# LordLiang/DrawingSpinUp

Hardware: AMD Instinct MI355X
Metric: drawings/sec end-to-end (512x512, 6 views, 24 frames) (higher is better)
Workload: dtype f16 (diffusion) / f16 table + f32 MLP (NSR) / f32 (stage-1 deformable convolutions, IS-Net, contour) / f32 with bf16 x 3 products (stage-2 convolutions; the reference: cuDNN TF32)

## Files before the change

drawingspinup_amd/_lib.py:

```python
import ctypes as C
import os

import torch

_HERE = os.path.dirname(os.path.abspath(__file__))
LIB_PATH = os.environ.get("DSU_HIP_LIB") or os.path.join(_HERE, "libdsu_hip.so")
MAX_LEVELS = 16

c_i32, c_i64, c_u32, c_f32, c_vp = C.c_int32, C.c_int64, C.c_uint32, C.c_float, C.c_void_p


class HashGridCfg(C.Structure):
    _fields_ = [("n_levels", c_u32), ("n_features", c_u32), ("log2_hashmap_size", c_u32),
                ("base_resolution", c_u32), ("per_level_scale", C.c_double)]


class HashGridLevels(C.Structure):
    _fields_ = [("offsets", c_u32 * (MAX_LEVELS + 1)), ("resolution", c_u32 * MAX_LEVELS),
                ("scale", c_f32 * MAX_LEVELS), ("hashed", c_u32 * MAX_LEVELS)]


class SdfMlp(C.Structure):
    _fields_ = [("w0", c_vp), ("b0", c_vp), ("w1", c_vp), ("b1", c_vp)]

# ... 158 lines not shown
    "dsu_nsr_driver_sync": [c_vp],
    "dsu_nsr_driver_timing": [c_vp, c_i32],
    "dsu_nsr_driver_timing_read": [c_vp, c_i32, C.POINTER(c_i64), C.POINTER(C.c_double),
                                   C.POINTER(C.c_double)],
    "dsu_nsr_driver_timing_flops": [c_vp, c_i32, C.POINTER(C.c_double)],
    "dsu_spatial_sort": [P, c_i64, c_f32, c_i32, P, P, P, c_i64, P],
    "dsu_spatial_sort_workspace_bytes": [c_i64, c_i32],
    "dsu_ray_aabb": [P, P, c_i64, P, P, c_f32, P, P, P],
    "dsu_ray_march_count": [P, P, P, P, c_i64, P, P, c_i32, c_f32, P, P],
    "dsu_ray_march_fill": [P, P, P, P, c_i64, P, P, c_i32, c_f32, P, P, P, P, P],
    "dsu_ray_march_scratch": [P, P, P, P, c_i64, P, P, c_i32, c_f32, c_i32, P, P, P, P],
    "dsu_ray_compact": [P, P, c_i32, P, P, c_i64, P, P, P, P],
    "dsu_ray_compact_points": [P, P, c_i32, P, P, c_i64, P, P, P, P, P, P],
    "dsu_ray_compact_points_cap": [P, P, c_i32, P, P, c_i64, P, P, P, P, P, c_i64, P],
    "dsu_points_tail": [P, c_i64, P, P, P, c_i64, c_f32, P],
    "dsu_spatial_sort_dev": [P, c_i64, P, c_i64, c_f32, c_i32, P, P, P, c_i64, P],
    "dsu_ray_offsets": [P, c_i64, P, P, P],
    "dsu_ortho_ray_batch": [P, P, P, c_i64, P, P, P, P, c_i32, P, P, P, c_i32, c_i32, P, P, P, P, P,
                            P, P],
    "dsu_ortho_ray_batch_split": [P, P, P, c_i64, P, P, P, P, c_i32, P, P, P, c_i32, c_i32, P, P, P, P, P,
                            P, P, P, P],
    "dsu_ray_losses": [P, P, P, P, P, P, c_i32, C.POINTER(RayLossCfg), P, P, P],
    "dsu_sample_losses": [P, P, c_i64, c_i64, c_f32, c_f32, c_f32, c_f32, c_i32, P, P, P, P],
    "dsu_texture_fwd": [C.POINTER(TexMlp), P, c_i64, P, P],
    "dsu_texture_bwd_workspace_bytes": [c_i64],
    "dsu_texture_bwd": [C.POINTER(TexMlp), P, P, P, c_i64, P, P, P, P, P, P, P, P, c_i64, P],
    "dsu_texture_fwd_shaded": [C.POINTER(TexMlp), P, P, c_i64, P, P, P],
    "dsu_texture_bwd_shaded": [C.POINTER(TexMlp), P, P, P, P, P, c_i64, c_i64, P, P, P, P, P, P, P, P,
                               P, c_i64, P],
    "dsu_weights_from_alpha_fwd": [P, P, P, c_i64, P, P],
    "dsu_weights_from_alpha_bwd": [P, P, P, P, P, c_i64, P, P],
    "dsu_accumulate_fwd": [P, P, c_i32, P, P, c_i64, P, P],
    "dsu_neus_composite_fwd": [P, P, P, P, P, P, P, P, c_i64, P, c_f32, P, P, P, P],
    "dsu_neus_composite_bwd": [P, P, P, P, P, P, P, P, c_i64, P, c_f32, P, P, P, P, P, P, P,
                               P, P],
    "dsu_shade_prep_fwd": [P, P, c_i64, P, P, P],
    "dsu_shade_prep_bwd": [P, P, P, c_i64, P, P, P],
    "dsu_shade_prep_bwd_tail": [P, P, P, c_i64, c_i64, P, P, P],
    "dsu_occgrid_ema": [P, P, P, c_i64, c_f32, P, P],
    "dsu_occgrid_binarize": [P, c_i64, c_f32, P, P],
    "dsu_ric_offsets": [c_i32, c_i32, P, P],
    "dsu_deform_conv3x3_fwd": [P, P, c_i64, P, c_i32, c_i32, c_i32, c_i32, c_i32, c_i32, P, P,
                               c_i32, P, P, P],
    "dsu_mv_attention_fwd": [P, P, P, P, P, c_i32, c_i32, c_i32, c_i32, c_i32, c_i32,
                             C.POINTER(c_i64), C.POINTER(c_i64), C.POINTER(c_i64),
                             C.POINTER(c_i64), c_f32, P],
# ... 113 lines not shown
```

drawingspinup_amd/csrc/nsr_driver.hip:

```cpp
#include "common.h"
#include "adamw_dev.h"

#include <math.h>
#include <string.h>

#include <mutex>
#include <vector>

namespace {

constexpr int N_GEO = 64 * 23 + 64 + 13 * 64 + 13;
constexpr int N_TEX = 64 * 16 + 64 + 64 * 64 + 64 + 3 * 64 + 3;
constexpr int N_SMALL = (64 * 23 + 64 + 64) + (13 * 64 + 13 + 13) + N_TEX + 1;

__device__ __forceinline__ uint4 philox(uint4 c, uint2 k) {
#pragma unroll
  for (int i = 0; i < 10; ++i) {
    const uint32_t hi0 = __umulhi(0xD2511F53u, c.x), lo0 = 0xD2511F53u * c.x;
    const uint32_t hi1 = __umulhi(0xCD9E8D57u, c.z), lo1 = 0xCD9E8D57u * c.z;
    c = make_uint4(hi1 ^ c.y ^ k.x, lo1, hi0 ^ c.w ^ k.y, lo0);
    k.x += 0x9E3779B9u;
    k.y += 0xBB67AE85u;
  }
  return c;
// ... 38 lines not shown
  float* variance;
  float* g_geo;
  float* g_tex;
  float* d_inv;
  float *m, *v;
  float *w0_eff, *w1_eff, *inv_s;
  float* zero_terms;
  const float* terms;
  float* terms_out;
  float lr_geo, lr_tex, lr_var, beta1, beta2, eps, wd, bc1, bc2_sqrt;
  int32_t update;
};

__device__ __forceinline__ void adamw_elem(float& x, float g, float& m, float& v, float lr,
                                           const SmallArgs& a) {
  const float omb1 = (float)(1.0 - (double)a.beta1), omb2 = (float)(1.0 - (double)a.beta2);
  x -= lr * a.wd * x;
  m = m + (g - m) * omb1;
  v = a.beta2 * v + omb2 * g * g;
  const float denom = sqrtf(v) / a.bc2_sqrt + a.eps;
  x -= (lr / a.bc1) * m / denom;
}

__global__ __launch_bounds__(1024) void small_update_kernel(SmallArgs a, dsu_table_adamw_args ta) {
  if (blockIdx.x > 0) {
    dsu_table_adamw_range(ta, (int64_t)(blockIdx.x - 1) * 1024 + threadIdx.x,
                          (int64_t)(gridDim.x - 1) * 1024);
    return;
  }
  __shared__ float s_g[N_GEO];
  __shared__ float s_v0[64 * 23], s_v1[13 * 64];
  __shared__ float s_gain[77], s_norm[77], s_dot[77];
  const int t = threadIdx.x;
  for (int i = t; i < 64 * 23; i += 1024) s_v0[i] = a.w0_v[i];
  for (int i = t; i < 13 * 64; i += 1024) s_v1[i] = a.w1_v[i];
  if (t < 77) s_gain[t] = t < 64 ? a.w0_g[t] : a.w1_g[t - 64];
  if (a.update)
    for (int i = t; i < N_GEO; i += 1024) s_g[i] = a.g_geo[i];
  __syncthreads();
  if (a.update) {
    if (t < 77) {
      const bool l0 = t < 64;
      const int r = l0 ? t : t - 64, cols = l0 ? 23 : 64;
      const float* vrow = (l0 ? s_v0 : s_v1) + r * cols;
      const float* grow = (l0 ? s_g : s_g + 64 * 23 + 64) + r * cols;
      float nn = 0.0f, dot = 0.0f;
      for (int c = 0; c < cols; ++c) {
        nn += vrow[c] * vrow[c];
        dot += grow[c] * vrow[c];
      }
      s_norm[t] = sqrtf(nn);
      s_dot[t] = dot;
    }
    __syncthreads();
    int off = 0;
    for (int i = t; i < 64 * 23; i += 1024) {
      const int r = i / 23;
      const float nrm = s_norm[r];
      const float g = (s_gain[r] / nrm) * (s_g[i] - s_v0[i] * s_dot[r] / (nrm * nrm));
      float x = s_v0[i], m = a.m[off + i], v = a.v[off + i];
      adamw_elem(x, g, m, v, a.lr_geo, a);
      a.w0_v[i] = x; a.m[off + i] = m; a.v[off + i] = v;
      s_v0[i] = x;
    }
    off += 64 * 23;
    float new_gain = 0.0f;
    if (t < 64) {
      float x = s_gain[t], m = a.m[off + t], v = a.v[off + t];
      adamw_elem(x, s_dot[t] / s_norm[t], m, v, a.lr_geo, a);
      a.w0_g[t] = x; a.m[off + t] = m; a.v[off + t] = v;
      new_gain = x;
    }
    off += 64;
    if (t < 64) {
      float x = a.b0[t], m = a.m[off + t], v = a.v[off + t];
      adamw_elem(x, s_g[64 * 23 + t], m, v, a.lr_geo, a);
      a.b0[t] = x; a.m[off + t] = m; a.v[off + t] = v;
    }
    off += 64;
    for (int i = t; i < 13 * 64; i += 1024) {
      const int r = i / 64;
      const float nrm = s_norm[64 + r];
      const float g = (s_gain[64 + r] / nrm) *
                      (s_g[64 * 23 + 64 + i] - s_v1[i] * s_dot[64 + r] / (nrm * nrm));
      float x = s_v1[i], m = a.m[off + i], v = a.v[off + i];
      adamw_elem(x, g, m, v, a.lr_geo, a);
      a.w1_v[i] = x; a.m[off + i] = m; a.v[off + i] = v;
      s_v1[i] = x;
    }
    off += 13 * 64;
    float new_gain1 = 0.0f;
    if (t < 13) {
      float x = s_gain[64 + t], m = a.m[off + t], v = a.v[off + t];
      adamw_elem(x, s_dot[64 + t] / s_norm[64 + t], m, v, a.lr_geo, a);
      a.w1_g[t] = x; a.m[off + t] = m; a.v[off + t] = v;
      new_gain1 = x;
    }
    off += 13;
    if (t < 13) {
      float x = a.b1[t], m = a.m[off + t], v = a.v[off + t];
      adamw_elem(x, s_g[64 * 23 + 64 + 13 * 64 + t], m, v, a.lr_geo, a);
      a.b1[t] = x; a.m[off + t] = m; a.v[off + t] = v;
    }
    off += 13;
    const int tn[6] = {64 * 16, 64, 64 * 64, 64, 3 * 64, 3};
    int go = 0;
    for (int k = 0; k < 6; ++k) {
      float* p = a.tex[k];
      for (int i = t; i < tn[k]; i += 1024) {
        float x = p[i], m = a.m[off + i], v = a.v[off + i];
        adamw_elem(x, a.g_tex[go + i], m, v, a.lr_tex, a);
        p[i] = x; a.m[off + i] = m; a.v[off + i] = v;
      }
      off += tn[k];
      go += tn[k];
    }
    if (t == 1023) {
      float x = a.variance[0], m = a.m[off], v = a.v[off];
      const float g = a.d_inv[0] * expf(x * 10.0f) * 10.0f;
      adamw_elem(x, g, m, v, a.lr_var, a);
      a.variance[0] = x; a.m[off] = m; a.v[off] = v;
      a.inv_s[0] = expf(x * 10.0f);
      a.d_inv[0] = 0.0f;
    }
    if (t < 3) a.zero_terms[t] = 0.0f;
    if (t >= 8 && t < 16 && a.terms_out) a.terms_out[t - 8] = a.terms[t - 8];
    __syncthreads();
    if (t < 64) s_gain[t] = new_gain;
    if (t < 13) s_gain[64 + t] = new_gain1;
    for (int i = t; i < N_GEO; i += 1024) a.g_geo[i] = 0.0f;
    for (int i = t; i < N_TEX; i += 1024) a.g_tex[i] = 0.0f;
    __syncthreads();
  } else if (t == 1023) {
    a.inv_s[0] = expf(a.variance[0] * 10.0f);
  }
  if (t < 77) {
    const bool l0 = t < 64;
    const int r = l0 ? t : t - 64, cols = l0 ? 23 : 64;
    const float* vrow = (l0 ? s_v0 : s_v1) + r * cols;
    float nn = 0.0f;
    for (int c = 0; c < cols; ++c) nn += vrow[c] * vrow[c];
    s_norm[t] = s_gain[t] / sqrtf(nn);
  }
  __syncthreads();
  for (int i = t; i < 64 * 23; i += 1024) a.w0_eff[i] = s_v0[i] * s_norm[i / 23];
  for (int i = t; i < 13 * 64; i += 1024) a.w1_eff[i] = s_v1[i] * s_norm[64 + i / 64];
}

struct Carve {
  char* base;
  int64_t off = 0;
  template <typename T>
  T* take(int64_t count) {
    off = (off + 255) / 256 * 256;
    T* p = base ? reinterpret_cast<T*>(base + off) : nullptr;
    off += count * (int64_t)sizeof(T);
    return p;
// ... 245 lines not shown
  sa.lr_geo = sa.lr_tex = sa.lr_var = 0.0f;
  sa.bc1 = sa.bc2_sqrt = 1.0f;
  if (update) {
    sa.lr_geo = a->lr_geometry; sa.lr_tex = a->lr_texture; sa.lr_var = a->lr_variance;
    sa.bc1 = (float)(1.0 - pow((double)c.beta1, (double)a->adam_step));
    sa.bc2_sqrt = (float)sqrt(1.0 - pow((double)c.beta2, (double)a->adam_step));
  }
  dsu_table_adamw_args ta{};
  int table_blocks = 0;
  if (update && a->table_p && !d->fold) {
    DSU_TRY(dsu_table_adamw(a->table_p, a->table_grad, a->table_m, a->table_v,
                            const_cast<void*>(a->table_img), a->table_n, a->table_lr, c.beta1, c.beta2,
                            a->table_eps, a->table_wd, a->table_bc1, a->table_bc2_sqrt, s));
  } else if (update && a->table_p) {
    if (a->table_n < 0 || (a->table_n & 3) || !a->table_grad || !a->table_m || !a->table_v ||
        !a->table_img || !(a->table_bc1 > 0.0f) || !(a->table_bc2_sqrt > 0.0f))
      return DSU_EINVAL;
    ta = dsu_table_adamw_args{(float4*)a->table_p, (float4*)a->table_grad, (float4*)a->table_m,
                              (float4*)a->table_v, (__half2*)const_cast<void*>(a->table_img),
                              a->table_n / 4, a->table_lr, c.beta1, c.beta2, a->table_eps,
                              a->table_wd, a->table_bc1, a->table_bc2_sqrt};
    table_blocks = (int)((ta.n4 + 1023) / 1024 < 512 ? (ta.n4 + 1023) / 1024 : 512);
  }
  small_update_kernel<<<dim3(1 + table_blocks), dim3(1024), 0, s>>>(sa, ta);
  DSU_CHECK_LAUNCH();
  return DSU_OK;
}

}

extern "C" {

int dsu_nsr_draws(uint64_t seed, int64_t step, int32_t n_rays, int32_t V, int32_t H, int32_t W,
                  int64_t* index, int64_t* x, int64_t* y, float* jitter, int32_t n_random,
                  float* pts_random, float* perturb, void* stream) {
  if (n_rays < 0 || n_random < 0 || V < 1 || H < 1 || W < 1 ||
      (n_rays && (!index || !x || !y || !jitter)) || (n_random && (!pts_random || !perturb)))
    return DSU_EINVAL;
  const int n = n_rays > n_random ? n_rays : n_random;
  if (n == 0) return DSU_OK;
  nsr_draw_kernel<<<dim3((n + 255) / 256), dim3(256), 0, (hipStream_t)stream>>>(
      seed, step, n_rays, V, H, W, index, x, y, jitter, n_random, pts_random, perturb);
  DSU_CHECK_LAUNCH();
  return DSU_OK;
}

int64_t dsu_nsr_driver_workspace_bytes(const dsu_nsr_driver_cfg* cfg) {
// ... 169 lines not shown
  if (d->timing) { d->work[0] += alg_bytes; d->flops[0] += fwd_flops; }
  if (a->prefetch_next && d->pack_gate == 1) {
    const int q = (int)((a->step + 1) % 3);
    dsu_nsr_step_args na = *a;
    na.inj_index = na.inj_x = na.inj_y = nullptr;
    na.inj_jitter = na.inj_pts_random = na.inj_perturb = nullptr;
    na.inj_rays = nullptr;
    DSU_HIP(hipEventRecord(d->fwd_done, s));
    DSU_HIP(hipStreamWaitEvent(d->side, d->fwd_done, 0));
    DSU_TRY(enqueue_pack(d, q, next_rays, na, false, d->side));
    DSU_HIP(hipEventRecord(d->ready[q], d->side));
    d->pf_valid[q] = true;
  }
  if (n_s > 0) {
    dsu_tex_mlp tex{c.tex[0], c.tex[1], c.tex[2], c.tex[3], c.tex[4], c.tex[5]};
    DSU_TRY(dsu_texture_fwd_shaded_m(&tex, L.a_feat, L.a_grad, n_s, L.normal, L.rgb,
                                     d->tex_masks ? L.tex_mask : nullptr, s));
    DSU_TRY(dsu_neus_composite_fwd(L.a_sdf, L.normal, L.rgb, f.rays_d, f.t_starts, f.t_ends,
                                   f.offsets, f.counts, a->n_rays, L.inv_s, a->cos_anneal_ratio,
                                   L.alpha, L.w, L.comp, s));
  } else {
    DSU_HIP(hipMemsetAsync(L.comp, 0, (size_t)a->n_rays * 8 * sizeof(float), s));
  }
  DSU_TRY(dsu_ray_losses(L.comp, f.rgb, f.normal, f.mask, f.cosines, f.vw, a->n_rays, &c.ray_loss,
                         terms, L.d_comp, s));
  dsu_partial_reduce tex_red{};
  bool have_tex_red = false;
  if (n_s > 0) {
    DSU_TRY(dsu_neus_composite_bwd(L.a_sdf, L.normal, L.rgb, f.rays_d, f.t_starts, f.t_ends,
                                   f.offsets, f.counts, a->n_rays, L.inv_s, a->cos_anneal_ratio,
                                   L.alpha, L.w, L.d_comp, nullptr, L.d_sdf_all, L.d_normal, L.d_rgb,
                                   L.d_inv, s));
    dsu_tex_mlp tex{c.tex[0], c.tex[1], c.tex[2], c.tex[3], c.tex[4], c.tex[5]};
    if (!d->fold) {
      float* gt = L.g_tex;
      DSU_TRY(dsu_texture_bwd_shaded(&tex, L.a_feat, L.a_grad, L.rgb, L.d_rgb, L.d_normal, n_s, 2 * n_r,
                                     L.d_grad_all, L.d_feat_all, gt, gt + 1024, gt + 1088, gt + 5184,
                                     gt + 5248, gt + 5440, L.tex_ws, L.tex_ws_bytes, s));
    } else {
    DSU_TRY(dsu_texture_bwd_shaded_partials_m(&tex, L.a_feat, L.a_grad, L.rgb, L.d_rgb, L.d_normal, n_s,
                                              2 * n_r, L.d_grad_all, L.d_feat_all,
                                              d->tex_masks ? L.tex_mask : nullptr, L.tex_ws,
                                              L.tex_ws_bytes, &tex_red, s));
    tex_red.map = L.tex_map;
    tex_red.base = L.g_tex;
    have_tex_red = true;
    }
  } else {
    DSU_HIP(hipMemsetAsync(L.d_feat_all, 0, (size_t)(2 * n_r) * 13 * sizeof(float), s));
  }
  DSU_TRY(dsu_sample_losses(L.a_sdf, L.a_grad, n_s, n_r, c.lambda_eikonal, c.lambda_sparsity,
                            c.sparsity_scale, c.lambda_smooth, 1 | 2, L.d_sdf_all, L.d_grad_all,
                            terms + 4, s));
  float* gg = L.g_geo;
  DSU_TRY(mark(d, 1, s));
  DSU_TRY(dsu_sdf_fd_bwd_sorted_fold(&c.grid, a->table_img, &mlp, pts, perm, n_all, c.radius, a->eps,
                                     a->active_levels, L.d_sdf_all, L.d_grad_all, L.d_feat_all, nullptr,
                                     a->table_grad, gg, gg + 64 * 23, gg + 64 * 23 + 64,
                                     gg + 64 * 23 + 64 + 13 * 64, L.sdf_ws, L.sdf_ws_bytes,
                                     L.enc_cache, d->gate, have_tex_red ? &tex_red : nullptr, s));
  DSU_TRY(mark(d, 1, s));
  if (d->timing) { d->work[1] += alg_bytes; d->flops[1] += bwd_flops; }
  if (a->prefetch_next && d->pack_gate == 2) {
    const int q = (int)((a->step + 1) % 3);
    dsu_nsr_step_args na = *a;
    na.inj_index = na.inj_x = na.inj_y = nullptr;
    na.inj_jitter = na.inj_pts_random = na.inj_perturb = nullptr;
    na.inj_rays = nullptr;
    DSU_HIP(hipStreamWaitEvent(d->side, d->gate, 0));
    DSU_TRY(enqueue_pack(d, q, next_rays, na, false, d->side));
    DSU_HIP(hipEventRecord(d->ready[q], d->side));
    d->pf_valid[q] = true;
  }
  DSU_TRY(launch_small_update(d, a, 1, s));
  d->last_step = a->step;
  guard.ok = true;
// ... 68 lines not shown
```

drawingspinup_amd/csrc/nsr_step.hip:

```cpp
#include "common.h"
#include "adamw_dev.h"
#include <math.h>

namespace {

constexpr int RL_THREADS = 1024;

__device__ __forceinline__ uint32_t flipf(float f) {
  const uint32_t u = __float_as_uint(f);
  return (u & 0x80000000u) ? ~u : (u | 0x80000000u);
}
__device__ __forceinline__ float unflipf(uint32_t k) {
  return __uint_as_float((k & 0x80000000u) ? (k & 0x7fffffffu) : ~k);
}

__device__ __forceinline__ float wave_sum(float v) {
#pragma unroll
  for (int o = 32; o > 0; o >>= 1) v += __shfl_xor(v, o);
  return v;
}
__device__ __forceinline__ int wave_sum_i(int v) {
#pragma unroll
  for (int o = 32; o > 0; o >>= 1) v += __shfl_xor(v, o);
  return v;
// ... 29 lines not shown
  }
  *total = all;
  return before + inc - v;
}

__device__ void bitonic_sort(uint64_t* keys, int P) {
  for (int k = 2; k <= P; k <<= 1) {
    for (int j = k >> 1; j > 0; j >>= 1) {
      for (int t = threadIdx.x; t < (P >> 1); t += blockDim.x) {
        const int i = ((t & ~(j - 1)) << 1) | (t & (j - 1));
        const int l = i | j;
        const uint64_t a = keys[i], b = keys[l];
        const bool up = (i & k) == 0;
        if ((a > b) == up) {
          keys[i] = b;
          keys[l] = a;
        }
      }
      __syncthreads();
    }
  }
}

struct RankLds {
  uint64_t* keys;
  int* pos;
  float* gerr;
  float* redf;
  int* redi;
};

template <class ErrF>
__device__ float rank_select(ErrF errf, const float* __restrict__ vw, int R, int P, double ratio,
                             bool mean, const RankLds& lds, int64_t* k_out) {
  for (int i = threadIdx.x; i < P; i += blockDim.x) {
    float e = 0.0f;
    bool valid = false;
    if (i < R) errf(i, e, valid);
    lds.keys[i] = ((uint64_t)flipf(valid ? e : INFINITY) << 32) | (uint32_t)i;
    lds.pos[i] = valid ? 1 : 0;
    lds.gerr[i] = 0.0f;
  }
  __syncthreads();
  const int E = P / blockDim.x;
  int c = 0;
  for (int q = 0; q < E; ++q) c += lds.pos[threadIdx.x * E + q];
  int nvalid;
  int run = block_excl_scan(c, lds.redi, &nvalid);
  for (int q = 0; q < E; ++q) {
    const int i = threadIdx.x * E + q;
    run += lds.pos[i];
    lds.pos[i] = run - 1;
  }
  __syncthreads();
  bitonic_sort(lds.keys, P);
  const int64_t kk = (int64_t)floor(ratio * (double)nvalid);
  float total = 0.0f;
  for (int64_t j = threadIdx.x; j < kk; j += blockDim.x) {
    const uint32_t idx = (uint32_t)lds.keys[j];
    int pj = lds.pos[idx];
    pj = pj < 0 ? 0 : pj;
    const uint64_t kt = lds.keys[pj];
    const float val = unflipf((uint32_t)(kt >> 32));
    const float w = vw ? vw[idx] : 1.0f;
    total += val * w;
    atomicAdd(&lds.gerr[(uint32_t)kt], w);
  }
  total = block_sum(total, lds.redf);
  *k_out = kk;
  return mean ? total / (float)kk : total;
}

__device__ __forceinline__ float signf0(float x) { return x > 0.0f ? 1.0f : (x < 0.0f ? -1.0f : 0.0f); }

__global__ __launch_bounds__(RL_THREADS) void ray_losses_kernel(
    const float* __restrict__ comp, const float* __restrict__ rgb, const float* __restrict__ normal,
    const float* __restrict__ maskf, const float* __restrict__ cosines,
    const float* __restrict__ vw, int R, int P, dsu_ray_loss_cfg cfg, float* __restrict__ terms,
    float* __restrict__ d_comp) {
  extern __shared__ __attribute__((aligned(16))) unsigned char smem[];
  RankLds lds;
  lds.keys = reinterpret_cast<uint64_t*>(smem);
  lds.pos = reinterpret_cast<int*>(smem + (size_t)P * 8);
  lds.gerr = reinterpret_cast<float*>(smem + (size_t)P * 12);
  lds.redf = reinterpret_cast<float*>(smem + (size_t)P * 16);
  lds.redi = reinterpret_cast<int*>(smem + (size_t)P * 16 + 128);
  const int term = blockIdx.x;

  auto fg = [&](int i) {
    const float cb = cosines[i] > -0.1f ? 0.0f : cosines[i];
    return maskf[i] > 0.0f && cb < -0.1f;
  };

  if (term == 0) {
    auto mse = [&](int i, float& e, bool& valid) {
      const float d0 = comp[i * 8 + 2] - rgb[i * 3], d1 = comp[i * 8 + 3] - rgb[i * 3 + 1],
                  d2 = comp[i * 8 + 4] - rgb[i * 3 + 2];
      e = (d0 * d0 + d1 * d1) + d2 * d2;
      valid = fg(i);
    };
    int64_t kk;
    float t = rank_select(mse, nullptr, R, P, cfg.rgb_p_ratio, true, lds, &kk) * cfg.lambda_rgb_mse;
    if (threadIdx.x == 0) terms[0] = t;
    __syncthreads();
    const float c = kk > 0 ? cfg.lambda_rgb_mse / (float)kk : 0.0f;
    for (int i = threadIdx.x; i < R; i += blockDim.x) {
      const float g = lds.gerr[i] * c;
#pragma unroll
      for (int ch = 0; ch < 3; ++ch)
        d_comp[i * 8 + 2 + ch] = 2.0f * (comp[i * 8 + 2 + ch] - rgb[i * 3 + ch]) * g;
    }
    float t1 = 0.0f;
    if (cfg.lambda_rgb_l1 != 0.0f) {
      __syncthreads();
      auto l1 = [&](int i, float& e, bool& valid) {
        const float d0 = comp[i * 8 + 2] - rgb[i * 3], d1 = comp[i * 8 + 3] - rgb[i * 3 + 1],
                    d2 = comp[i * 8 + 4] - rgb[i * 3 + 2];
        e = (fabsf(d0) + fabsf(d1)) + fabsf(d2);
        valid = fg(i);
      };
      t1 = rank_select(l1, nullptr, R, P, cfg.rgb_p_ratio, true, lds, &kk) * cfg.lambda_rgb_l1;
      __syncthreads();
      const float c1 = kk > 0 ? cfg.lambda_rgb_l1 / (float)kk : 0.0f;
      for (int i = threadIdx.x; i < R; i += blockDim.x) {
        const float g = lds.gerr[i] * c1;
#pragma unroll
        for (int ch = 0; ch < 3; ++ch)
          d_comp[i * 8 + 2 + ch] += signf0(comp[i * 8 + 2 + ch] - rgb[i * 3 + ch]) * g;
      }
    }
    if (threadIdx.x == 0) terms[1] = t1;
  } else if (term == 1) {
    float S = 1.0f;
    if (cfg.geo_aware) {
      float s = 0.0f;
      for (int i = threadIdx.x; i < R; i += blockDim.x) {
        const float cb = cosines[i] > -0.1f ? 0.0f : cosines[i];
        s += expf(fabsf(cb));
      }
      S = block_sum(s, lds.redf);
      __syncthreads();
    }
    auto cosim = [&](int i, float& cs, float u[3], float gh[3], float& nn, float& a, float n[3]) {
      const float v0 = comp[i * 8 + 5], v1 = comp[i * 8 + 6], v2 = comp[i * 8 + 7];
      const float nv = sqrtf((v0 * v0 + v1 * v1) + v2 * v2);
      a = fmaxf(nv, 1e-12f);
      n[0] = v0 / a; n[1] = v1 / a; n[2] = v2 / a;
      nn = fmaxf(sqrtf((n[0] * n[0] + n[1] * n[1]) + n[2] * n[2]), 1e-8f);
      const float g0 = normal[i * 3], g1 = normal[i * 3 + 1], g2 = normal[i * 3 + 2];
      const float gn = fmaxf(sqrtf((g0 * g0 + g1 * g1) + g2 * g2), 1e-8f);
      u[0] = n[0] / nn; u[1] = n[1] / nn; u[2] = n[2] / nn;
      gh[0] = g0 / gn; gh[1] = g1 / gn; gh[2] = g2 / gn;
      cs = (u[0] * gh[0] + u[1] * gh[1]) + u[2] * gh[2];
    };
    auto nerr = [&](int i, float& e, bool& valid) {
      float cs, u[3], gh[3], nn, a, n[3];
      cosim(i, cs, u, gh, nn, a, n);
      e = 1.0f - cs;
      if (cfg.geo_aware) {
        const float cb = cosines[i] > -0.1f ? 0.0f : cosines[i];
        e = e * expf(fabsf(cb)) / S;
      }
      valid = fg(i);
    };
    int64_t kk;
    const bool mean = !cfg.geo_aware;
    float t = rank_select(nerr, vw, R, P, cfg.normal_p_ratio, mean, lds, &kk) * cfg.lambda_normal;
    if (threadIdx.x == 0) terms[2] = t;
    __syncthreads();
    const float c = mean ? (kk > 0 ? cfg.lambda_normal / (float)kk : 0.0f) : cfg.lambda_normal;
    for (int i = threadIdx.x; i < R; i += blockDim.x) {
      float cs, u[3], gh[3], nn, a, n[3];
      cosim(i, cs, u, gh, nn, a, n);
      float de = lds.gerr[i] * c;
      if (cfg.geo_aware) {
        const float cb = cosines[i] > -0.1f ? 0.0f : cosines[i];
        de = de / S * expf(fabsf(cb));
      }
      const float dcs = -de;
      const float nv = sqrtf((comp[i * 8 + 5] * comp[i * 8 + 5] + comp[i * 8 + 6] * comp[i * 8 + 6]) +
                             comp[i * 8 + 7] * comp[i * 8 + 7]);
      float dv[3] = {0.0f, 0.0f, 0.0f};
      if (nv > 1e-12f && dcs != 0.0f) {
        float tn[3];
#pragma unroll
        for (int ch = 0; ch < 3; ++ch) tn[ch] = (gh[ch] - cs * u[ch]) / nn * dcs;
        const float nt = (n[0] * tn[0] + n[1] * tn[1]) + n[2] * tn[2];
#pragma unroll
        for (int ch = 0; ch < 3; ++ch) dv[ch] = (tn[ch] - n[ch] * nt) / a;
      }
      d_comp[i * 8 + 5] = dv[0];
      d_comp[i * 8 + 6] = dv[1];
      d_comp[i * 8 + 7] = dv[2];
    }
  } else {
    auto bce = [&](int i, float& e, bool& valid) {
      const float oc = fminf(fmaxf(comp[i * 8], 1e-3f), 1.0f - 1e-3f);
      const float m = maskf[i];
      e = -(m * logf(oc) + (1.0f - m) * logf(1.0f - oc));
      valid = true;
    };
    int64_t kk;
    float t = rank_select(bce, vw, R, P, cfg.mask_p_ratio, true, lds, &kk) * cfg.lambda_mask;
    if (threadIdx.x == 0) terms[3] = t;
    __syncthreads();
    const float c = kk > 0 ? cfg.lambda_mask / (float)kk : 0.0f;
    for (int i = threadIdx.x; i < R; i += blockDim.x) {
      const float o = comp[i * 8];
      const float oc = fminf(fmaxf(o, 1e-3f), 1.0f - 1e-3f);
      const float m = maskf[i];
      const bool pass = o >= 1e-3f && o <= 1.0f - 1e-3f;
      const float g = lds.gerr[i] * c;
      d_comp[i * 8] = pass ? g * (-(m / oc) + (1.0f - m) / (1.0f - oc)) : 0.0f;
      d_comp[i * 8 + 1] = 0.0f;
    }
  }
}

__global__ __launch_bounds__(256) void sample_losses_kernel(
    const float* __restrict__ sdf, const float* __restrict__ grad, int64_t n_s, int64_t n_r,
    float lambda_eik, float lambda_sp, float sp_scale, float lambda_sm, int accumulate_prefix,
    float* __restrict__ d_sdf, float* __restrict__ d_grad, float* __restrict__ terms) {
  float s_eik = 0.0f, s_sp = 0.0f, s_sm = 0.0f;
  const int64_t n = n_s + n_r;
  const float inv_ns = n_s > 0 ? 1.0f / (float)n_s : 0.0f;
  const float inv_nr = n_r > 0 ? 1.0f / (float)n_r : 0.0f;
  const float inv_3nr = n_r > 0 ? 1.0f / (float)(3 * n_r) : 0.0f;
  for (int64_t i = blockIdx.x * (int64_t)blockDim.x + threadIdx.x; i < n;
       i += (int64_t)gridDim.x * blockDim.x) {
    if (i < n_s) {
      const float g0 = grad[i * 3], g1 = grad[i * 3 + 1], g2 = grad[i * 3 + 2];
      const float nrm = sqrtf((g0 * g0 + g1 * g1) + g2 * g2);
      const float dl = nrm - 1.0f;
      s_eik += dl * dl;
      const float cf = nrm > 0.0f ? lambda_eik * 2.0f * dl * inv_ns / nrm : 0.0f;
      if (accumulate_prefix) {
        d_grad[i * 3] += cf * g0;
        d_grad[i * 3 + 1] += cf * g1;
        d_grad[i * 3 + 2] += cf * g2;
// ... 231 lines not shown
      index, x, y, n, c2w, origins, directions, images, image_channels, normals, masks, view_weights,
      H, W, rays, rgb, normal, mask, cosines, vw, rays_o, rays_d);
  DSU_CHECK_LAUNCH();
  return DSU_OK;
}

int dsu_ray_losses(const float* comp, const float* rgb, const float* normal, const float* mask,
                   const float* cosines, const float* view_weights, int32_t n_rays,
                   const dsu_ray_loss_cfg* cfg, float* terms, float* d_comp, void* stream) {
  if (!cfg || !terms || n_rays < 0) return DSU_EINVAL;
  if (n_rays && (!comp || !rgb || !normal || !mask || !cosines || !view_weights || !d_comp))
    return DSU_EINVAL;
  if (n_rays > DSU_RAY_LOSS_MAX_RAYS) return DSU_EUNSUP;
  int P = RL_THREADS;
  while (P < n_rays) P <<= 1;
  const size_t shm = (size_t)P * 16 + 256;
  DSU_ENSURE_DYN_LDS(ray_losses_kernel, shm);
  ray_losses_kernel<<<3, RL_THREADS, shm, (hipStream_t)stream>>>(
      comp, rgb, normal, mask, cosines, view_weights, n_rays, P, *cfg, terms, d_comp);
  DSU_CHECK_LAUNCH();
  return DSU_OK;
}

int dsu_sample_losses(const float* sdf_all, const float* grad_all, int64_t n_samples,
                      int64_t n_random, float lambda_eikonal, float lambda_sparsity,
                      float sparsity_scale, float lambda_smooth, int32_t accumulate_prefix,
                      float* d_sdf_all, float* d_grad_all, float* terms, void* stream) {
  if (n_samples < 0 || n_random < 0 || !terms) return DSU_EINVAL;
  const int64_t n = n_samples + n_random;
  if (n && (!sdf_all || !grad_all || !d_sdf_all || !d_grad_all)) return DSU_EINVAL;
  hipStream_t s = (hipStream_t)stream;
  if (!(accumulate_prefix & 2) && hipMemsetAsync(terms, 0, 3 * sizeof(float), s) != hipSuccess)
    return DSU_ELAUNCH;
  if (n == 0) return DSU_OK;
  sample_losses_kernel<<<dsu_capped_blocks(n, 256, 512), 256, 0, s>>>(
      sdf_all, grad_all, n_samples, n_random, lambda_eikonal, lambda_sparsity, sparsity_scale,
      lambda_smooth, accumulate_prefix & 1, d_sdf_all, d_grad_all, terms);
  DSU_CHECK_LAUNCH();
  return DSU_OK;
}

int dsu_ray_offsets(const int32_t* counts, int64_t n_rays, int32_t* offsets, int32_t* stats,
                    void* stream) {
  if (n_rays < 0 || !stats || (n_rays && (!counts || !offsets))) return DSU_EINVAL;
  ray_offsets_kernel<<<1, 1024, 0, (hipStream_t)stream>>>(counts, n_rays, offsets, stats);
  DSU_CHECK_LAUNCH();
// ... 5 lines not shown
```

include/dsu_hip.h:

```cpp
#ifndef DSU_HIP_H
#define DSU_HIP_H

#include <stdint.h>

#ifdef __cplusplus
extern "C" {
#endif

#define DSU_OK 0
#define DSU_EINVAL (-1)
#define DSU_ELAUNCH (-2)
#define DSU_EUNSUP (-3)

#define DSU_MAX_LEVELS 16

const char* dsu_strerror(int code);
int dsu_ab_switches(void);
int dsu_abi_version(void);
int dsu_set_onewave_grid_cap(int32_t workgroups);
int dsu_set_scatter_grid_cap(int32_t workgroups);
int dsu_set_nsr_side_stream_priority(int32_t level);
int dsu_set_nsr_side_stream_pooling(int32_t on);

typedef struct {
// ... 246 lines not shown

int dsu_ortho_ray_batch_split(const int64_t* index, const int64_t* x, const int64_t* y, int64_t n,
                              const float* c2w, const float* origins, const float* directions,
                              const float* images, int32_t image_channels, const float* normals,
                              const float* masks, const float* view_weights, int32_t H, int32_t W,
                              float* rays, float* rgb, float* normal, float* mask, float* cosines,
                              float* vw, float* rays_o, float* rays_d, void* stream);

#define DSU_RAY_LOSS_MAX_RAYS 8192
typedef struct dsu_ray_loss_cfg {
  double rgb_p_ratio, normal_p_ratio, mask_p_ratio;
  float lambda_rgb_mse, lambda_rgb_l1, lambda_normal, lambda_mask;
  int32_t geo_aware;
  int32_t reserved;
} dsu_ray_loss_cfg;
int dsu_ray_losses(const float* comp, const float* rgb, const float* normal, const float* mask,
                   const float* cosines, const float* view_weights, int32_t n_rays,
                   const dsu_ray_loss_cfg* cfg, float* terms, float* d_comp, void* stream);

int dsu_sample_losses(const float* sdf_all, const float* grad_all, int64_t n_samples,
                      int64_t n_random, float lambda_eikonal, float lambda_sparsity,
                      float sparsity_scale, float lambda_smooth, int32_t accumulate_prefix,
                      float* d_sdf_all, float* d_grad_all, float* terms, void* stream);


int dsu_ric_offsets(int32_t H, int32_t W, float* offsets, void* stream);

int dsu_deform_conv3x3_fwd(const float* input, const float* offset, int64_t offset_batch_stride,
                           const float* weight, int32_t B, int32_t C, int32_t H, int32_t W,
                           int32_t O, int32_t in_relu, const float* ep_scale,
                           const float* ep_shift, int32_t act, const float* residual, float* out,
                           void* stream);

int dsu_conv2d_fwd(const float* input, const float* weight, const float* bias, int32_t B,
                   int32_t C, int32_t H, int32_t W, int32_t O, int32_t k, int32_t stride,
                   int32_t pad, int32_t in_relu, const float* ep_scale, const float* ep_shift,
                   int32_t act, const float* residual, float* out, void* stream);

int64_t dsu_conv_x3_packed_elems(int32_t O, int32_t C, int32_t k);
int dsu_conv_x3_pack_weights(const float* weight, int32_t O, int32_t C, int32_t k, uint16_t* w_hi,
                             uint16_t* w_mid, void* stream);
int dsu_deform_conv3x3_fwd_x3(const float* input, const float* offset, int64_t offset_batch_stride,
                              const uint16_t* w_hi, const uint16_t* w_mid, int32_t B, int32_t C,
                              int32_t H, int32_t W, int32_t O, int32_t in_relu,
                              const float* ep_scale, const float* ep_shift, int32_t act,
                              const float* residual, float* out, void* stream);
// ... 275 lines not shown
```

Baseline: 0.3435.

## Fuse sample losses into ray-loss kernel and split optimizer update across blocks

The sparsity and smoothness sample-loss terms now run in extra blocks of the ray-loss kernel, saving one launch. The eikonal gradient moves into a small elementwise add kernel that runs after the texture backward. Ray-loss ranking uses a bitonic sort that replaces block barriers with wavefront barriers once the compare distance fits inside one wave. The small-parameter AdamW kernel moves the texture-MLP and variance updates into a second block and prefetches the moment tensors into registers, which shortens the serial critical path of block 0 at the cost of one more launched block and more register use.

```diff
diff --git a/drawingspinup_amd/_lib.py b/drawingspinup_amd/_lib.py
--- a/drawingspinup_amd/_lib.py
+++ b/drawingspinup_amd/_lib.py
@@ -204,6 +204,9 @@
                             P, P, P, P],
     "dsu_ray_losses": [P, P, P, P, P, P, c_i32, C.POINTER(RayLossCfg), P, P, P],
     "dsu_sample_losses": [P, P, c_i64, c_i64, c_f32, c_f32, c_f32, c_f32, c_i32, P, P, P, P],
+    "dsu_ray_sample_losses": [P, P, P, P, P, P, c_i32, C.POINTER(RayLossCfg), P, P, P, P, c_i64, c_i64,
+                              c_f32, c_f32, c_f32, c_f32, P, P, P, P],
+    "dsu_eikonal_grad_add": [P, c_i64, c_f32, P, P],
     "dsu_texture_fwd": [C.POINTER(TexMlp), P, c_i64, P, P],
     "dsu_texture_bwd_workspace_bytes": [c_i64],
     "dsu_texture_bwd": [C.POINTER(TexMlp), P, P, P, c_i64, P, P, P, P, P, P, P, P, c_i64, P],
diff --git a/drawingspinup_amd/csrc/nsr_driver.hip b/drawingspinup_amd/csrc/nsr_driver.hip
--- a/drawingspinup_amd/csrc/nsr_driver.hip
+++ b/drawingspinup_amd/csrc/nsr_driver.hip
@@ -84,16 +84,84 @@
   x -= (lr / a.bc1) * m / denom;
 }
 
+constexpr int TEX_PER_THREAD = (N_TEX + 1023) / 1024;
+
 __global__ __launch_bounds__(1024) void small_update_kernel(SmallArgs a, dsu_table_adamw_args ta) {
-  if (blockIdx.x > 0) {
-    dsu_table_adamw_range(ta, (int64_t)(blockIdx.x - 1) * 1024 + threadIdx.x,
-                          (int64_t)(gridDim.x - 1) * 1024);
+  if (blockIdx.x > 1) {
+    dsu_table_adamw_range(ta, (int64_t)(blockIdx.x - 2) * 1024 + threadIdx.x,
+                          (int64_t)(gridDim.x - 2) * 1024);
+    return;
+  }
+  const int t = threadIdx.x;
+  constexpr int OFF_W0G = 64 * 23, OFF_B0 = OFF_W0G + 64, OFF_W1V = OFF_B0 + 64,
+                OFF_W1G = OFF_W1V + 13 * 64, OFF_B1 = OFF_W1G + 13, OFF_TEX = OFF_B1 + 13,
+                OFF_VAR = OFF_TEX + N_TEX;
+  if (blockIdx.x == 1) {
+    if (!a.update) {
+      if (t == 1023) a.inv_s[0] = expf(a.variance[0] * 10.0f);
+      return;
+    }
+    const int tn[6] = {64 * 16, 64, 64 * 64, 64, 3 * 64, 3};
+    float* px[TEX_PER_THREAD];
+    float x[TEX_PER_THREAD], g[TEX_PER_THREAD], m[TEX_PER_THREAD], v[TEX_PER_THREAD];
+#pragma unroll
+    for (int q = 0; q < TEX_PER_THREAD; ++q) {
+      const int e = t + 1024 * q;
+      px[q] = nullptr;
+      int start = 0;
+#pragma unroll
+      for (int k = 0; k < 6; ++k) {
+        if (e >= start && e < start + tn[k]) px[q] = a.tex[k] + (e - start);
+        start += tn[k];
+      }
+      if (px[q]) {
+        x[q] = *px[q]; g[q] = a.g_tex[e]; m[q] = a.m[OFF_TEX + e]; v[q] = a.v[OFF_TEX + e];
+      }
+    }
+    float var_x = 0.0f, var_m = 0.0f, var_v = 0.0f, var_d = 0.0f, term_in = 0.0f;
+    if (t == 1023) { var_x = a.variance[0]; var_m = a.m[OFF_VAR]; var_v = a.v[OFF_VAR]; var_d = a.d_inv[0]; }
+    if (t >= 8 && t < 16 && a.terms_out) term_in = a.terms[t - 8];
+#pragma unroll
+    for (int q = 0; q < TEX_PER_THREAD; ++q) {
+      if (!px[q]) continue;
+      const int e = t + 1024 * q;
+      adamw_elem(x[q], g[q], m[q], v[q], a.lr_tex, a);
+      *px[q] = x[q]; a.m[OFF_TEX + e] = m[q]; a.v[OFF_TEX + e] = v[q];
+      a.g_tex[e] = 0.0f;
+    }
+    if (t == 1023) {
+      const float gv = var_d * expf(var_x * 10.0f) * 10.0f;
+      adamw_elem(var_x, gv, var_m, var_v, a.lr_var, a);
+      a.variance[0] = var_x; a.m[OFF_VAR] = var_m; a.v[OFF_VAR] = var_v;
+      a.inv_s[0] = expf(var_x * 10.0f);
+      a.d_inv[0] = 0.0f;
+    }
+    if (t < 3) a.zero_terms[t] = 0.0f;
+    if (t >= 8 && t < 16 && a.terms_out) a.terms_out[t - 8] = term_in;
     return;
   }
   __shared__ float s_g[N_GEO];
   __shared__ float s_v0[64 * 23], s_v1[13 * 64];
   __shared__ float s_gain[77], s_norm[77], s_dot[77];
-  const int t = threadIdx.x;
+  float m0[2] = {0.0f, 0.0f}, v0[2] = {0.0f, 0.0f};
+  float m_g0 = 0.0f, v_g0 = 0.0f, m_b0 = 0.0f, v_b0 = 0.0f, x_b0 = 0.0f;
+  float m1 = 0.0f, v1 = 0.0f, m_g1 = 0.0f, v_g1 = 0.0f, m_b1 = 0.0f, v_b1 = 0.0f, x_b1 = 0.0f;
+  if (a.update) {
+#pragma unroll
+    for (int q = 0; q < 2; ++q) {
+      const int i = t + 1024 * q;
+      if (i < 64 * 23) { m0[q] = a.m[i]; v0[q] = a.v[i]; }
+    }
+    if (t < 64) {
+      m_g0 = a.m[OFF_W0G + t]; v_g0 = a.v[OFF_W0G + t];
+      m_b0 = a.m[OFF_B0 + t]; v_b0 = a.v[OFF_B0 + t]; x_b0 = a.b0[t];
+    }
+    if (t < 13 * 64) { m1 = a.m[OFF_W1V + t]; v1 = a.v[OFF_W1V + t]; }
+    if (t < 13) {
+      m_g1 = a.m[OFF_W1G + t]; v_g1 = a.v[OFF_W1G + t];
+      m_b1 = a.m[OFF_B1 + t]; v_b1 = a.v[OFF_B1 + t]; x_b1 = a.b1[t];
+    }
+  }
   for (int i = t; i < 64 * 23; i += 1024) s_v0[i] = a.w0_v[i];
   for (int i = t; i < 13 * 64; i += 1024) s_v1[i] = a.w1_v[i];
   if (t < 77) s_gain[t] = t < 64 ? a.w0_g[t] : a.w1_g[t - 64];
@@ -101,6 +169,7 @@
     for (int i = t; i < N_GEO; i += 1024) s_g[i] = a.g_geo[i];
   __syncthreads();
   if (a.update) {
+    for (int i = t; i < N_GEO; i += 1024) a.g_geo[i] = 0.0f;
     if (t < 77) {
       const bool l0 = t < 64;
       const int r = l0 ? t : t - 64, cols = l0 ? 23 : 64;
@@ -115,86 +184,55 @@
       s_dot[t] = dot;
     }
     __syncthreads();
-    int off = 0;
-    for (int i = t; i < 64 * 23; i += 1024) {
-      const int r = i / 23;
-      const float nrm = s_norm[r];
-      const float g = (s_gain[r] / nrm) * (s_g[i] - s_v0[i] * s_dot[r] / (nrm * nrm));
-      float x = s_v0[i], m = a.m[off + i], v = a.v[off + i];
-      adamw_elem(x, g, m, v, a.lr_geo, a);
-      a.w0_v[i] = x; a.m[off + i] = m; a.v[off + i] = v;
-      s_v0[i] = x;
-    }
-    off += 64 * 23;
+#pragma unroll
+    for (int q = 0; q < 2; ++q) {
+      const int i = t + 1024 * q;
+      if (i < 64 * 23) {
+        const int r = i / 23;
+        const float nrm = s_norm[r];
+        const float g = (s_gain[r] / nrm) * (s_g[i] - s_v0[i] * s_dot[r] / (nrm * nrm));
+        float x = s_v0[i];
+        adamw_elem(x, g, m0[q], v0[q], a.lr_geo, a);
+        a.w0_v[i] = x; a.m[i] = m0[q]; a.v[i] = v0[q];
+        s_v0[i] = x;
+      }
+    }
     float new_gain = 0.0f;
     if (t < 64) {
-      float x = s_gain[t], m = a.m[off + t], v = a.v[off + t];
-      adamw_elem(x, s_dot[t] / s_norm[t], m, v, a.lr_geo, a);
-      a.w0_g[t] = x; a.m[off + t] = m; a.v[off + t] = v;
+      float x = s_gain[t];
+      adamw_elem(x, s_dot[t] / s_norm[t], m_g0, v_g0, a.lr_geo, a);
+      a.w0_g[t] = x; a.m[OFF_W0G + t] = m_g0; a.v[OFF_W0G + t] = v_g0;
       new_gain = x;
     }
-    off += 64;
     if (t < 64) {
-      float x = a.b0[t], m = a.m[off + t], v = a.v[off + t];
-      adamw_elem(x, s_g[64 * 23 + t], m, v, a.lr_geo, a);
-      a.b0[t] = x; a.m[off + t] = m; a.v[off + t] = v;
-    }
-    off += 64;
-    for (int i = t; i < 13 * 64; i += 1024) {
-      const int r = i / 64;
+      adamw_elem(x_b0, s_g[64 * 23 + t], m_b0, v_b0, a.lr_geo, a);
+      a.b0[t] = x_b0; a.m[OFF_B0 + t] = m_b0; a.v[OFF_B0 + t] = v_b0;
+    }
+    if (t < 13 * 64) {
+      const int i = t, r = i / 64;
       const float nrm = s_norm[64 + r];
       const float g = (s_gain[64 + r] / nrm) *
                       (s_g[64 * 23 + 64 + i] - s_v1[i] * s_dot[64 + r] / (nrm * nrm));
-      float x = s_v1[i], m = a.m[off + i], v = a.v[off + i];
-      adamw_elem(x, g, m, v, a.lr_geo, a);
-      a.w1_v[i] = x; a.m[off + i] = m; a.v[off + i] = v;
+      float x = s_v1[i];
+      adamw_elem(x, g, m1, v1, a.lr_geo, a);
+      a.w1_v[i] = x; a.m[OFF_W1V + i] = m1; a.v[OFF_W1V + i] = v1;
       s_v1[i] = x;
     }
-    off += 13 * 64;
     float new_gain1 = 0.0f;
     if (t < 13) {
-      float x = s_gain[64 + t], m = a.m[off + t], v = a.v[off + t];
-      adamw_elem(x, s_dot[64 + t] / s_norm[64 + t], m, v, a.lr_geo, a);
-      a.w1_g[t] = x; a.m[off + t] = m; a.v[off + t] = v;
+      float x = s_gain[64 + t];
+      adamw_elem(x, s_dot[64 + t] / s_norm[64 + t], m_g1, v_g1, a.lr_geo, a);
+      a.w1_g[t] = x; a.m[OFF_W1G + t] = m_g1; a.v[OFF_W1G + t] = v_g1;
       new_gain1 = x;
     }
-    off += 13;
     if (t < 13) {
-      float x = a.b1[t], m = a.m[off + t], v = a.v[off + t];
-      adamw_elem(x, s_g[64 * 23 + 64 + 13 * 64 + t], m, v, a.lr_geo, a);
-      a.b1[t] = x; a.m[off + t] = m; a.v[off + t] = v;
-    }
-    off += 13;
-    const int tn[6] = {64 * 16, 64, 64 * 64, 64, 3 * 64, 3};
-    int go = 0;
-    for (int k = 0; k < 6; ++k) {
-      float* p = a.tex[k];
-      for (int i = t; i < tn[k]; i += 1024) {
-        float x = p[i], m = a.m[off + i], v = a.v[off + i];
-        adamw_elem(x, a.g_tex[go + i], m, v, a.lr_tex, a);
-        p[i] = x; a.m[off + i] = m; a.v[off + i] = v;
-      }
-      off += tn[k];
-      go += tn[k];
-    }
-    if (t == 1023) {
-      float x = a.variance[0], m = a.m[off], v = a.v[off];
-      const float g = a.d_inv[0] * expf(x * 10.0f) * 10.0f;
-      adamw_elem(x, g, m, v, a.lr_var, a);
-      a.variance[0] = x; a.m[off] = m; a.v[off] = v;
-      a.inv_s[0] = expf(x * 10.0f);
-      a.d_inv[0] = 0.0f;
-    }
-    if (t < 3) a.zero_terms[t] = 0.0f;
-    if (t >= 8 && t < 16 && a.terms_out) a.terms_out[t - 8] = a.terms[t - 8];
+      adamw_elem(x_b1, s_g[64 * 23 + 64 + 13 * 64 + t], m_b1, v_b1, a.lr_geo, a);
+      a.b1[t] = x_b1; a.m[OFF_B1 + t] = m_b1; a.v[OFF_B1 + t] = v_b1;
+    }
     __syncthreads();
     if (t < 64) s_gain[t] = new_gain;
     if (t < 13) s_gain[64 + t] = new_gain1;
-    for (int i = t; i < N_GEO; i += 1024) a.g_geo[i] = 0.0f;
-    for (int i = t; i < N_TEX; i += 1024) a.g_tex[i] = 0.0f;
     __syncthreads();
-  } else if (t == 1023) {
-    a.inv_s[0] = expf(a.variance[0] * 10.0f);
   }
   if (t < 77) {
     const bool l0 = t < 64;
@@ -486,7 +524,7 @@
                               a->table_wd, a->table_bc1, a->table_bc2_sqrt};
     table_blocks = (int)((ta.n4 + 1023) / 1024 < 512 ? (ta.n4 + 1023) / 1024 : 512);
   }
-  small_update_kernel<<<dim3(1 + table_blocks), dim3(1024), 0, s>>>(sa, ta);
+  small_update_kernel<<<dim3(2 + table_blocks), dim3(1024), 0, s>>>(sa, ta);
   DSU_CHECK_LAUNCH();
   return DSU_OK;
 }
@@ -702,8 +740,10 @@
   } else {
     DSU_HIP(hipMemsetAsync(L.comp, 0, (size_t)a->n_rays * 8 * sizeof(float), s));
   }
-  DSU_TRY(dsu_ray_losses(L.comp, f.rgb, f.normal, f.mask, f.cosines, f.vw, a->n_rays, &c.ray_loss,
-                         terms, L.d_comp, s));
+  DSU_TRY(dsu_ray_sample_losses(L.comp, f.rgb, f.normal, f.mask, f.cosines, f.vw, a->n_rays,
+                                &c.ray_loss, terms, L.d_comp, L.a_sdf, L.a_grad, n_s, n_r,
+                                c.lambda_eikonal, c.lambda_sparsity, c.sparsity_scale, c.lambda_smooth,
+                                L.d_sdf_all, L.d_grad_all, terms + 4, s));
   dsu_partial_reduce tex_red{};
   bool have_tex_red = false;
   if (n_s > 0) {
@@ -729,9 +769,7 @@
   } else {
     DSU_HIP(hipMemsetAsync(L.d_feat_all, 0, (size_t)(2 * n_r) * 13 * sizeof(float), s));
   }
-  DSU_TRY(dsu_sample_losses(L.a_sdf, L.a_grad, n_s, n_r, c.lambda_eikonal, c.lambda_sparsity,
-                            c.sparsity_scale, c.lambda_smooth, 1 | 2, L.d_sdf_all, L.d_grad_all,
-                            terms + 4, s));
+  DSU_TRY(dsu_eikonal_grad_add(L.a_grad, n_s, c.lambda_eikonal, L.d_grad_all, s));
   float* gg = L.g_geo;
   DSU_TRY(mark(d, 1, s));
   DSU_TRY(dsu_sdf_fd_bwd_sorted_fold(&c.grid, a->table_img, &mlp, pts, perm, n_all, c.radius, a->eps,
diff --git a/drawingspinup_amd/csrc/nsr_step.hip b/drawingspinup_amd/csrc/nsr_step.hip
--- a/drawingspinup_amd/csrc/nsr_step.hip
+++ b/drawingspinup_amd/csrc/nsr_step.hip
@@ -75,6 +75,32 @@
   }
 }
 
+__device__ __forceinline__ void wave_lds_sync() {
+  __builtin_amdgcn_fence(__ATOMIC_RELEASE, "wavefront");
+  __builtin_amdgcn_wave_barrier();
+  __builtin_amdgcn_fence(__ATOMIC_ACQUIRE, "wavefront");
+}
+
+__device__ void bitonic_sort_wave_local(uint64_t* keys, int P) {
+  for (int k = 2; k <= P; k <<= 1) {
+    for (int j = k >> 1; j > 0; j >>= 1) {
+      for (int t = threadIdx.x; t < (P >> 1); t += blockDim.x) {
+        const int i = ((t & ~(j - 1)) << 1) | (t & (j - 1));
+        const int l = i | j;
+        const uint64_t a = keys[i], b = keys[l];
+        const bool up = (i & k) == 0;
+        if ((a > b) == up) {
+          keys[i] = b;
+          keys[l] = a;
+        }
+      }
+      const int next = j > 1 ? (j >> 1) : k;
+      if (j <= 64 && next <= 64) wave_lds_sync();
+      else __syncthreads();
+    }
+  }
+}
+
 struct RankLds {
   uint64_t* keys;
   int* pos;
@@ -83,7 +109,7 @@
   int* redi;
 };
 
-template <class ErrF>
+template <bool WAVE_LOCAL, class ErrF>
 __device__ float rank_select(ErrF errf, const float* __restrict__ vw, int R, int P, double ratio,
                              bool mean, const RankLds& lds, int64_t* k_out) {
   for (int i = threadIdx.x; i < P; i += blockDim.x) {
@@ -106,7 +132,8 @@
     lds.pos[i] = run - 1;
   }
   __syncthreads();
-  bitonic_sort(lds.keys, P);
+  if (WAVE_LOCAL) bitonic_sort_wave_local(lds.keys, P);
+  else bitonic_sort(lds.keys, P);
   const int64_t kk = (int64_t)floor(ratio * (double)nvalid);
   float total = 0.0f;
   for (int64_t j = threadIdx.x; j < kk; j += blockDim.x) {
@@ -126,19 +153,19 @@
 
 __device__ __forceinline__ float signf0(float x) { return x > 0.0f ? 1.0f : (x < 0.0f ? -1.0f : 0.0f); }
 
-__global__ __launch_bounds__(RL_THREADS) void ray_losses_kernel(
+template <bool WAVE_LOCAL>
+__device__ __forceinline__ void ray_loss_term(
+    const int term, unsigned char* smem,
     const float* __restrict__ comp, const float* __restrict__ rgb, const float* __restrict__ normal,
     const float* __restrict__ maskf, const float* __restrict__ cosines,
-    const float* __restrict__ vw, int R, int P, dsu_ray_loss_cfg cfg, float* __restrict__ terms,
+    const float* __restrict__ vw, int R, int P, const dsu_ray_loss_cfg& cfg, float* __restrict__ terms,
     float* __restrict__ d_comp) {
-  extern __shared__ __attribute__((aligned(16))) unsigned char smem[];
   RankLds lds;
   lds.keys = reinterpret_cast<uint64_t*>(smem);
   lds.pos = reinterpret_cast<int*>(smem + (size_t)P * 8);
   lds.gerr = reinterpret_cast<float*>(smem + (size_t)P * 12);
   lds.redf = reinterpret_cast<float*>(smem + (size_t)P * 16);
   lds.redi = reinterpret_cast<int*>(smem + (size_t)P * 16 + 128);
-  const int term = blockIdx.x;
 
   auto fg = [&](int i) {
     const float cb = cosines[i] > -0.1f ? 0.0f : cosines[i];
@@ -153,7 +180,7 @@
       valid = fg(i);
     };
     int64_t kk;
-    float t = rank_select(mse, nullptr, R, P, cfg.rgb_p_ratio, true, lds, &kk) * cfg.lambda_rgb_mse;
+    float t = rank_select<WAVE_LOCAL>(mse, nullptr, R, P, cfg.rgb_p_ratio, true, lds, &kk) * cfg.lambda_rgb_mse;
     if (threadIdx.x == 0) terms[0] = t;
     __syncthreads();
     const float c = kk > 0 ? cfg.lambda_rgb_mse / (float)kk : 0.0f;
@@ -172,7 +199,7 @@
         e = (fabsf(d0) + fabsf(d1)) + fabsf(d2);
         valid = fg(i);
       };
-      t1 = rank_select(l1, nullptr, R, P, cfg.rgb_p_ratio, true, lds, &kk) * cfg.lambda_rgb_l1;
+      t1 = rank_select<WAVE_LOCAL>(l1, nullptr, R, P, cfg.rgb_p_ratio, true, lds, &kk) * cfg.lambda_rgb_l1;
       __syncthreads();
       const float c1 = kk > 0 ? cfg.lambda_rgb_l1 / (float)kk : 0.0f;
       for (int i = threadIdx.x; i < R; i += blockDim.x) {
@@ -218,7 +245,7 @@
     };
     int64_t kk;
     const bool mean = !cfg.geo_aware;
-    float t = rank_select(nerr, vw, R, P, cfg.normal_p_ratio, mean, lds, &kk) * cfg.lambda_normal;
+    float t = rank_select<WAVE_LOCAL>(nerr, vw, R, P, cfg.normal_p_ratio, mean, lds, &kk) * cfg.lambda_normal;
     if (threadIdx.x == 0) terms[2] = t;
     __syncthreads();
     const float c = mean ? (kk > 0 ? cfg.lambda_normal / (float)kk : 0.0f) : cfg.lambda_normal;
@@ -254,7 +281,7 @@
       valid = true;
     };
     int64_t kk;
-    float t = rank_select(bce, vw, R, P, cfg.mask_p_ratio, true, lds, &kk) * cfg.lambda_mask;
+    float t = rank_select<WAVE_LOCAL>(bce, vw, R, P, cfg.mask_p_ratio, true, lds, &kk) * cfg.lambda_mask;
     if (threadIdx.x == 0) terms[3] = t;
     __syncthreads();
     const float c = kk > 0 ? cfg.lambda_mask / (float)kk : 0.0f;
@@ -268,6 +295,100 @@
       d_comp[i * 8 + 1] = 0.0f;
     }
   }
+}
+
+__global__ __launch_bounds__(RL_THREADS) void ray_losses_kernel(
+    const float* __restrict__ comp, const float* __restrict__ rgb, const float* __restrict__ normal,
+    const float* __restrict__ maskf, const float* __restrict__ cosines,
+    const float* __restrict__ vw, int R, int P, dsu_ray_loss_cfg cfg, float* __restrict__ terms,
+    float* __restrict__ d_comp) {
+  extern __shared__ __attribute__((aligned(16))) unsigned char smem[];
+  ray_loss_term<false>(blockIdx.x, smem, comp, rgb, normal, maskf, cosines, vw, R, P, cfg, terms, d_comp);
+}
+
+struct SampleTermArgs {
+  const float *sdf, *grad;
+  int64_t n_s, n_r;
+  float lambda_eik, lambda_sp, sp_scale, lambda_sm;
+  float *d_sdf, *d_grad, *terms;
+};
+
+__device__ __forceinline__ void sample_terms_tail(const SampleTermArgs& a, int first, int count,
+                                                  float* red ) {
+  float s_eik = 0.0f, s_sp = 0.0f, s_sm = 0.0f;
+  const int64_t n = a.n_s + a.n_r;
+  const float inv_ns = a.n_s > 0 ? 1.0f / (float)a.n_s : 0.0f;
+  const float inv_nr = a.n_r > 0 ? 1.0f / (float)a.n_r : 0.0f;
+  const float inv_3nr = a.n_r > 0 ? 1.0f / (float)(3 * a.n_r) : 0.0f;
+  for (int64_t i = first * (int64_t)blockDim.x + threadIdx.x; i < n; i += (int64_t)count * blockDim.x) {
+    if (i < a.n_s) {
+      const float g0 = a.grad[i * 3], g1 = a.grad[i * 3 + 1], g2 = a.grad[i * 3 + 2];
+      const float nrm = sqrtf((g0 * g0 + g1 * g1) + g2 * g2);
+      const float dl = nrm - 1.0f;
+      s_eik += dl * dl;
+    } else {
+      const int64_t p = i, q = i + a.n_r;
+      const float x = a.sdf[p];
+      const float ex = expf(-a.sp_scale * fabsf(x));
+      s_sp += ex;
+      a.d_sdf[p] = a.lambda_sp * inv_nr * ex * (-a.sp_scale) * signf0(x);
+      a.d_sdf[q] = 0.0f;
+#pragma unroll
+      for (int c = 0; c < 3; ++c) {
+        const float df = a.grad[p * 3 + c] - a.grad[q * 3 + c];
+        s_sm += fabsf(df);
+        const float sg = a.lambda_sm * inv_3nr * signf0(df);
+        a.d_grad[p * 3 + c] = sg;
+        a.d_grad[q * 3 + c] = -sg;
+      }
+    }
+  }
+  s_eik = wave_sum(s_eik);
+  s_sp = wave_sum(s_sp);
+  s_sm = wave_sum(s_sm);
+  const int lane = threadIdx.x & 63, wave = threadIdx.x >> 6, nw = blockDim.x >> 6;
+  if (lane == 0) {
+    red[wave] = s_eik;
+    red[16 + wave] = s_sp;
+    red[32 + wave] = s_sm;
+  }
+  __syncthreads();
+  if (threadIdx.x < 3) {
+    float t = 0.0f;
+    for (int w = 0; w < nw; ++w) t += red[16 * threadIdx.x + w];
+    const float sc = threadIdx.x == 0 ? inv_ns * a.lambda_eik
+                                      : (threadIdx.x == 1 ? inv_nr * a.lambda_sp : inv_3nr * a.lambda_sm);
+    if (t != 0.0f) atomicAdd(&a.terms[threadIdx.x], t * sc);
+  }
+}
+
+__global__ __launch_bounds__(RL_THREADS) void ray_sample_losses_kernel(
+    const float* __restrict__ comp, const float* __restrict__ rgb, const float* __restrict__ normal,
+    const float* __restrict__ maskf, const float* __restrict__ cosines,
+    const float* __restrict__ vw, int R, int P, dsu_ray_loss_cfg cfg, float* __restrict__ terms,
+    float* __restrict__ d_comp, SampleTermArgs sa) {
+  extern __shared__ __attribute__((aligned(16))) unsigned char smem[];
+  if (blockIdx.x >= 3) {
+    sample_terms_tail(sa, (int)blockIdx.x - 3, (int)gridDim.x - 3, reinterpret_cast<float*>(smem));
+    return;
+  }
+  ray_loss_term<true>(blockIdx.x, smem, comp, rgb, normal, maskf, cosines, vw, R, P, cfg, terms, d_comp);
+}
+
+__global__ __launch_bounds__(256) void eikonal_grad_add_kernel(const float* __restrict__ grad,
+                                                               int64_t n_s, float lambda_eik,
+                                                               float* __restrict__ d_grad) {
+  const int64_t i = blockIdx.x * (int64_t)blockDim.x + threadIdx.x;
+  if (i >= n_s) return;
+  const float inv_ns = 1.0f / (float)n_s;
+  const float g0 = grad[i * 3], g1 = grad[i * 3 + 1], g2 = grad[i * 3 + 2];
+  const float e0 = d_grad[i * 3], e1 = d_grad[i * 3 + 1], e2 = d_grad[i * 3 + 2];
+  const float nrm = sqrtf((g0 * g0 + g1 * g1) + g2 * g2);
+  const float dl = nrm - 1.0f;
+  const float cf = nrm > 0.0f ? lambda_eik * 2.0f * dl * inv_ns / nrm : 0.0f;
+  d_grad[i * 3] = e0 + cf * g0;
+  d_grad[i * 3 + 1] = e1 + cf * g1;
+  d_grad[i * 3 + 2] = e2 + cf * g2;
 }
 
 __global__ __launch_bounds__(256) void sample_losses_kernel(
@@ -545,6 +666,42 @@
   return DSU_OK;
 }
 
+int dsu_ray_sample_losses(const float* comp, const float* rgb, const float* normal, const float* mask,
+                          const float* cosines, const float* view_weights, int32_t n_rays,
+                          const dsu_ray_loss_cfg* cfg, float* terms, float* d_comp,
+                          const float* sdf_all, const float* grad_all, int64_t n_samples,
+                          int64_t n_random, float lambda_eikonal, float lambda_sparsity,
+                          float sparsity_scale, float lambda_smooth, float* d_sdf_all,
+                          float* d_grad_all, float* sample_terms, void* stream) {
+  if (!cfg || !terms || !sample_terms || n_rays < 0 || n_samples < 0 || n_random < 0) return DSU_EINVAL;
+  if (n_rays && (!comp || !rgb || !normal || !mask || !cosines || !view_weights || !d_comp))
+    return DSU_EINVAL;
+  const int64_t n = n_samples + n_random;
+  if (n && (!sdf_all || !grad_all || !d_sdf_all || !d_grad_all)) return DSU_EINVAL;
+  if (n_rays > DSU_RAY_LOSS_MAX_RAYS) return DSU_EUNSUP;
+  int P = RL_THREADS;
+  while (P < n_rays) P <<= 1;
+  const size_t shm = (size_t)P * 16 + 256;
+  DSU_ENSURE_DYN_LDS(ray_sample_losses_kernel, shm);
+  const int extra = n ? dsu_capped_blocks(n, RL_THREADS, 128) : 0;
+  ray_sample_losses_kernel<<<3 + extra, RL_THREADS, shm, (hipStream_t)stream>>>(
+      comp, rgb, normal, mask, cosines, view_weights, n_rays, P, *cfg, terms, d_comp,
+      SampleTermArgs{sdf_all, grad_all, n_samples, n_random, lambda_eikonal, lambda_sparsity,
+                     sparsity_scale, lambda_smooth, d_sdf_all, d_grad_all, sample_terms});
+  DSU_CHECK_LAUNCH();
+  return DSU_OK;
+}
+
+int dsu_eikonal_grad_add(const float* grad_all, int64_t n_samples, float lambda_eikonal,
+                         float* d_grad_all, void* stream) {
+  if (n_samples < 0 || (n_samples && (!grad_all || !d_grad_all))) return DSU_EINVAL;
+  if (n_samples == 0) return DSU_OK;
+  eikonal_grad_add_kernel<<<dsu_blocks_for(n_samples, 256), 256, 0, (hipStream_t)stream>>>(
+      grad_all, n_samples, lambda_eikonal, d_grad_all);
+  DSU_CHECK_LAUNCH();
+  return DSU_OK;
+}
+
 int dsu_sample_losses(const float* sdf_all, const float* grad_all, int64_t n_samples,
                       int64_t n_random, float lambda_eikonal, float lambda_sparsity,
                       float sparsity_scale, float lambda_smooth, int32_t accumulate_prefix,
diff --git a/include/dsu_hip.h b/include/dsu_hip.h
--- a/include/dsu_hip.h
+++ b/include/dsu_hip.h
@@ -292,6 +292,16 @@
                       int64_t n_random, float lambda_eikonal, float lambda_sparsity,
                       float sparsity_scale, float lambda_smooth, int32_t accumulate_prefix,
                       float* d_sdf_all, float* d_grad_all, float* terms, void* stream);
+
+int dsu_ray_sample_losses(const float* comp, const float* rgb, const float* normal, const float* mask,
+                          const float* cosines, const float* view_weights, int32_t n_rays,
+                          const dsu_ray_loss_cfg* cfg, float* terms, float* d_comp,
+                          const float* sdf_all, const float* grad_all, int64_t n_samples,
+                          int64_t n_random, float lambda_eikonal, float lambda_sparsity,
+                          float sparsity_scale, float lambda_smooth, float* d_sdf_all,
+                          float* d_grad_all, float* sample_terms, void* stream);
+int dsu_eikonal_grad_add(const float* grad_all, int64_t n_samples, float lambda_eikonal,
+                         float* d_grad_all, void* stream);
 
 
 int dsu_ric_offsets(int32_t H, int32_t W, float* offsets, void* stream);
```

After: 0.3425 (median of 2 runs). No clear change (-0.3%).
